# StructuralNeurobiologyLab/SyConn

Measured on AMD Instinct MI355X. Metric: segmented Mvoxels/s (whole node), 128^3 EM tiles, higher is better.
Workload: dtype bf16; 1 GPU; BASELINE configs[1]: semseg_spine 3D U-Net on 128^3 uint8 tiles, 96 tiles per GPU per step in launch sets of 8 (sd_forward_labels_batch), random-init weights, HOST TO HOST: pinned host uint8 tiles -> H2D -> kernels -> pinned host uint8 labels (stored by the last kernel, no copy), 3 HIP streams, 2 buffer sets; tiles_per_launch_set=8, parallelism=tile-sharded x1, hip_streams_per_gpu=3, collective=none

## Files before the change

syconn_amd/csrc/sd_conv_mfma.h:

```cpp
#pragma once
#include "sd_internal.h"
#include "../../include/syconn_dense.h"
#include <algorithm>
#include <cstdlib>
#include <mutex>
#include <string>
#include <type_traits>
#include <utility>

#include "sd_device.h"


template <typename T>
__device__ __forceinline__ void store_tile_rows(typename Act<T>::v4 (&o)[4], T* base, size_t P, size_t vidx, bool valid,
                                                int cbase, int half, int Cd) {
    typedef __attribute__((ext_vector_type(2))) unsigned u2;
    typedef __attribute__((ext_vector_type(4))) unsigned u4;
    u2 a0 = __builtin_bit_cast(u2, o[0]), a1 = __builtin_bit_cast(u2, o[1]);
    u2 a2 = __builtin_bit_cast(u2, o[2]), a3 = __builtin_bit_cast(u2, o[3]);
    unsigned x;
    x = a0.x; { unsigned y = a1.x; swap32(x, y); a0.x = x; a1.x = y; }
    x = a0.y; { unsigned y = a1.y; swap32(x, y); a0.y = x; a1.y = y; }
    x = a2.x; { unsigned y = a3.x; swap32(x, y); a2.x = x; a3.x = y; }
    x = a2.y; { unsigned y = a3.y; swap32(x, y); a2.y = x; a3.y = y; }
// ... 36 lines not shown
#pragma unroll
    for (int q = 0; q < 4; ++q) {
        const int n = cbase + 4 * half + 8 * q;
        f32x4 b = {0.f, 0.f, 0.f, 0.f};
        if (n < Cd) b = *reinterpret_cast<const f32x4*>(bias + n);
#pragma unroll
        for (int e = 0; e < 4; ++e) {
            float v = acc[4 * q + e] + b[e];
            if (relu) v = fmaxf(v, 0.f);
            o[q][e] = (T)v;
        }
    }
    store_tile_rows<T>(o, base, P, vidx, valid, cbase, half, Cd);
}

template <typename T>
__device__ __forceinline__ typename Act<T>::v8 gn_apply8(typename Act<T>::v8 v, const float* sc, const float* sh, int relu) {
    typedef __attribute__((ext_vector_type(4))) unsigned u4;
    const f32x4 s0 = *reinterpret_cast<const f32x4*>(sc), s1 = *reinterpret_cast<const f32x4*>(sc + 4);
    const f32x4 t0 = *reinterpret_cast<const f32x4*>(sh), t1 = *reinterpret_cast<const f32x4*>(sh + 4);
#pragma unroll
    for (int e = 0; e < 4; ++e) {
        v[e] = (T)fmaf((float)v[e], s0[e], t0[e]);
        v[4 + e] = (T)fmaf((float)v[4 + e], s1[e], t1[e]);
    }
    if (relu) {
        u4 u = __builtin_bit_cast(u4, v);
        u.x = pk_max16(u.x, 0u); u.y = pk_max16(u.y, 0u); u.z = pk_max16(u.z, 0u); u.w = pk_max16(u.w, 0u);
        v = __builtin_bit_cast(typename Act<T>::v8, u);
    }
    return v;
}

template <int KZ, int WAVES, int MT> struct ConvGeo {
    static constexpr int BZ = KZ == 3 ? (WAVES / 4) * MT : 1;
    static constexpr int BY = KZ == 3 ? 8 : WAVES * 2 * MT;
    static constexpr int BX = 16;
};


constexpr int dma_count(int w, int waves, int a_instr, int j0, int j1) {
    int n = 0;
    for (int j = j0; j < j1; ++j) n += (w + j * waves < a_instr) ? 1 : 0;
    return n;
}
constexpr int zroll_wait(int nt, int u_want, int i_want) {
    int seq = 0;
    int wseq[9] = {0, 0, 0, 0, 0, 0, 0, 0, 0};
    int xseq[3][6] = {{0}};
    seq += nt; wseq[0] = seq - 1;
    for (int m = 0; m < 4; ++m) xseq[0][m] = seq++;
    for (int u = 0; u < 9; ++u) {
        const int kx = u / 3, kz = u % 3;
        if (u + 1 < 9) { seq += nt; wseq[u + 1] = seq - 1; }
        for (int i = 0; i < 4; ++i) {
            if (u == u_want && i == i_want) {
                int need = xseq[kx][i + kz];
                if (i == 0 && wseq[u] > need) need = wseq[u];
                return seq - 1 - need;
            }
            if (kz == 0 && i == 0) xseq[kx][4] = seq++;
            else if (kz == 1 && i == 0) xseq[kx][5] = seq++;
            else if (kz == 2 && kx < 2) xseq[kx + 1][i] = seq++;
        }
    }
    return 0;
}
template <typename T, int KZ, int NT, int WAVES, int NSLOT, int MT, int MODE>
__global__ __launch_bounds__(WAVES * 64, WAVES == 12 ? 3 : 2) void k_conv_mfma(const ConvParams p) {
    constexpr bool FF = MODE == 1 || MODE == 4 || MODE == 5, GN = MODE == 2, FU8 = MODE == 5;
    constexpr bool ZROLL = KZ == 3 && NT != 3;
    if (p.clk && blockIdx.x == 0 && threadIdx.x == 0) { p.clk[0] = __builtin_readcyclecounter(); p.clk[1] = __builtin_amdgcn_s_memrealtime(); }
    constexpr bool SP = MODE == 3 || MODE == 4;
    static_assert(!SP || std::is_same<T, f16_t>::value, "split plan: fp16 planes");
    constexpr bool LEAN = MT == 4 || NT == 3;
#ifndef SD_LATE_W
#define SD_LATE_W 1
#endif
#ifdef SD_NO_SPREAD
    constexpr bool SPREAD = false;
#else
    constexpr bool SPREAD = MT == 4 && KZ == 3 && WAVES == 8 && NSLOT == 0 && (MODE == 0 || MODE == 3);
#endif
    using v8 = typename Act<T>::v8;
    using G = ConvGeo<KZ, WAVES, MT>;
    constexpr bool WRES = NSLOT > 0;
    constexpr bool RING = NSLOT < 0;
    static_assert(!RING || (KZ == 1 && MODE == 0 && MT == 2 && NSLOT == -3), "ring form: planar, plain, 2 voxel tiles per wave");
    constexpr int NA = WRES ? NSLOT : RING ? -NSLOT : 2;
    constexpr int NW = RING ? -NSLOT : 2;
    constexpr int BZ = G::BZ, BY = G::BY, BX = G::BX;
    constexpr int PZ = KZ / 2;
    constexpr int HZ = BZ + KZ - 1, HY = BY + 2, HX = BX + 2;
    constexpr int NH = HZ * HY * HX;
    constexpr int A_INSTR = (NH * 2 + 63) / 64;
    constexpr int A_BYTES = A_INSTR * 1024;
    constexpr int B_INSTR = 9 * NT;
    constexpr int B_BYTES = B_INSTR * 1024;
    constexpr int SLICE = HY * HX * 32;
    constexpr int AJ = (A_INSTR + WAVES - 1) / WAVES;
    constexpr int WJ = (B_INSTR + WAVES - 1) / WAVES;
    constexpr int WAITN = WRES ? (NA - 2) * AJ : RING ? AJ + WJ : 0;
    static_assert(WAITN < 64, "vmcnt immediate");
    extern __shared__ __attribute__((aligned(16))) char smem[];
    const int nchunks = p.nchunk0 + p.nchunk1;
    const int nstages = nchunks * KZ;
    char* const ldsA = smem;
    char* const ldsB = smem + NA * A_BYTES;
    float* const wl = reinterpret_cast<float*>(ldsB + (WRES ? nstages : NW) * B_BYTES);
    char* const fwl = reinterpret_cast<char*>(wl) + SD_CONV_PARAM_BYTES;
    char* const ldsDummy = fwl + (p.final_wfrag ? NT * 4096 : 0);
    float* const fpatch = reinterpret_cast<float*>(ldsDummy + 1024);
    float* const gnl = fpatch;

    const int tid = threadIdx.x, lane = tid & 63;
    const int wave = __builtin_amdgcn_readfirstlane(tid >> 6);
    const int nsb = p.nbx * p.nby * p.nbz;
    const int nb = blockIdx.y;
    const int gsz = gridDim.x;

    int tzs[MT], tys[MT];
#pragma unroll
    for (int i = 0; i < MT; ++i) {
        if (KZ == 3) { tzs[i] = MT * (wave >> 2) + i; tys[i] = 2 * (wave & 3); }
        else { tzs[i] = 0; tys[i] = 2 * MT * wave + 2 * i; }
    }
    const int dy = (lane & 31) >> 4, dxl = lane & 15, half = lane >> 5;
    int xoffE[MT], xoffO[MT];
#pragma unroll
    for (int i = 0; i < MT; ++i) {
        const int hv = (tzs[i] * HY + tys[i] + dy) * HX + dxl;
        xoffE[i] = hv * 32 + ((half ^ (dy & 1)) << 4);
        xoffO[i] = hv * 32 + ((half ^ (dy & 1) ^ 1) << 4);
    }

    for (int idx = tid; idx < NT * 32; idx += WAVES * 64) {
        const int n = nb * NT * 32 + idx;
        wl[idx] = n < p.Cd ? p.bias[n] : 0.f;
    }
    if constexpr (GN) {
        const int per_tile = nchunks * 32;
        for (int i = tid; i < p.batch * per_tile; i += WAVES * 64) {
            const int t = i / per_tile, r = i - t * per_tile, c = r >> 5, e = r & 31, ch = e & 15, is_shift = e >> 4;
            const bool s0 = c < p.nchunk0;
            const float* const base = s0 ? p.gn0 : p.gn1;
            const int C = s0 ? p.C0 : p.C1, cc = s0 ? c : c - p.nchunk0;
            float v = is_shift ? 0.f : 1.f;
            if (base) v = reinterpret_cast<const float*>(reinterpret_cast<const char*>(base) + (size_t)t * p.tstride)[is_shift * C + cc * SD_CHUNK + ch];
            gnl[i] = v;
        }
    }
    if (p.final_wfrag) {
        if (tid < 8) wl[NT * 32 + tid] = tid < p.final_cout ? p.final_b[tid] : 0.f;
        const T* const fwp = reinterpret_cast<const T*>(p.final_wfrag);
        for (int k = wave; k < NT * 4; k += WAVES)
            *reinterpret_cast<v8*>(fwl + (k * 64 + lane) * 16) = *reinterpret_cast<const v8*>(fwp + ((size_t)k * 64 + lane) * 8);
    }
// ... 152 lines not shown
            }
        }
    };
    int sf_c = 0, sf_round = 0, sf_slot = 0, sf_z = 0, sf_y = 0, sf_x = 0, sf_t = 0;
    bool sf_ok = false;
    auto stream_block = [&]() {
        const int lbf = block_of(sf_round);
        sf_ok = lbf >= 0;
        if (sf_ok) coords(lbf, sf_z, sf_y, sf_x, sf_t);
    };
    auto dma_stream_next = [&]() {
        if (sf_c == 0) stream_block();
        dma_halo(sf_c, sf_slot, sf_z, sf_y, sf_x, sf_t, sf_ok);
        gn_note(sf_c, sf_slot, sf_z, sf_y, sf_x, sf_t, sf_ok);
        if (++sf_c == nchunks) { sf_c = 0; ++sf_round; }
        if (++sf_slot == NA) sf_slot = 0;
    };

    auto ring_issue = [&]() {
        if (sf_c == 0) stream_block();
        const char* src = wbase + (size_t)sf_c * B_BYTES + lane * 16;
        char* dst = ldsB + sf_slot * B_BYTES;
#pragma unroll
        for (int j = 0; j < WJ; ++j) {
            const int k = wave + j * WAVES;
            const bool inst = sf_ok && k < B_INSTR;
            glds16(inst ? src + k * 1024 : reinterpret_cast<const char*>(p.zero), inst ? dst + k * 1024 : ldsDummy);
        }
        dma_halo(sf_c, sf_slot, sf_z, sf_y, sf_x, sf_t, sf_ok);
        if (++sf_c == nchunks) { sf_c = 0; ++sf_round; }
        if (++sf_slot == NA) sf_slot = 0;
    };

#ifdef SD_TIMING
    long long tstamp[8];
    long long sstamp[16];
    int tcount = 0;
#define SD_T(i) do { if (tcount == SD_TB) tstamp[i] = __builtin_readcyclecounter(); } while (0)
#else
#define SD_T(i) do {} while (0)
#endif
#ifndef SD_TS
#define SD_TS 0
#endif
#ifndef SD_TB
#define SD_TB 2
#endif
    int lb = block_of(0);
    if (lb < 0) return;
    int z0, y0, x0, tn;
    coords(lb, z0, y0, x0, tn);

    constexpr int FPX = HX + 2, FPY = HY + 2, FNP = FPX * FPY, FPT = (FNP + WAVES * 64 - 1) / (WAVES * 64);
    float fpv[FF ? FPT : 1];
    auto patch_fetch = [&](int bz0, int by0, int bx0, int btile) {
#pragma unroll
        for (int k = 0; k < FPT; ++k) {
            const int i = tid + k * WAVES * 64;
            const int px = i % FPX, py = i / FPX;
            const int y = by0 - 2 + py, x = bx0 - 2 + px;
            float v = 0.f;
            if (i < FNP && (unsigned)bz0 < (unsigned)p.D && (unsigned)y < (unsigned)p.H && (unsigned)x < (unsigned)p.W) {
                const size_t idx = ((size_t)bz0 * p.H + y) * p.W + x;
                const char* const in = reinterpret_cast<const char*>(p.first_in) + (size_t)btile * p.first_in_tstride;
                if constexpr (FU8) v = __builtin_bit_cast(float, u8_bf16_pair(reinterpret_cast<const uint8_t*>(in)[idx]));
                else if (p.first_in_f32) v = reinterpret_cast<const float*>(in)[idx];
                else v = (float)reinterpret_cast<const uint8_t*>(in)[idx] / 255.0f;
            }
            fpv[k] = v;
        }
    };
    auto patch_park = [&](int buf) {
#pragma unroll
        for (int k = 0; k < FPT; ++k) {
            const int i = tid + k * WAVES * 64;
            if (i < FNP) fpatch[buf * FNP + i] = fpv[k];
        }
    };
    constexpr int NF1 = (FF && !SP && NA == 3) ? 2 : 1;
    float* const ffw = fpatch + 2 * FNP;
    if constexpr (FF) {
        patch_fetch(z0, y0, x0, tn);
        patch_park(0);
        if constexpr (FU8) {
            if (tid == 0) reinterpret_cast<unsigned*>(ffw)[0] = SD_BF16_ONE_PAIR;
            typedef __attribute__((ext_vector_type(4))) unsigned u4;
            for (int i = tid; i < NF1 * 2 * 64; i += WAVES * 64) reinterpret_cast<u4*>(ffw + 4)[i] = reinterpret_cast<const u4*>(p.first_w3)[i];
        } else
        for (int i = tid; i < NF1 * (5 * 64 + 32); i += WAVES * 64) ffw[i] = i < NF1 * 320 ? p.first_w[i] : p.first_bias[i - NF1 * 320];
    }
    if (WRES) {
        for (int s = 0; s < nstages; ++s) dma_weights(s, s);
        if (!FF) for (int f = 0; f < NA - 1; ++f) dma_stream_next();
    } else if (RING) {
        for (int f = 0; f < NA - 1; ++f) ring_issue();
    } else {
        dma_weights(0, 0);
        dma_halo(0, 0, z0, y0, x0, tn, true);
        gn_note(0, 0, z0, y0, x0, tn, true);
    }
    if constexpr (GN) {
        static_assert(!GN || WAITN == 0, "deferred GroupNorm apply: every halo DMA is awaited at its stage end");
        asm volatile("s_waitcnt vmcnt(0) lgkmcnt(0)\n\ts_barrier" ::: "memory");
        gn_transform();
        asm volatile("s_waitcnt lgkmcnt(0)\n\ts_barrier" ::: "memory");
    } else {
        asm volatile("s_waitcnt vmcnt(%0) lgkmcnt(0)\n\ts_barrier" ::"n"(WAITN) : "memory");
    }

    StoreGuard<T> sguard;
#ifndef SD_PRIO
#define SD_PRIO 2
#endif
    if constexpr (SPREAD && SD_PRIO != 0) {
        if ((SD_PRIO == 1) == (wave >= WAVES / 2)) asm volatile("s_setprio 1");
    }
    int gc = 0, gs = 0;
    int ph0 = 0;
    if constexpr (SPREAD) {
        const int hv0 = (wave * 64 + lane) >> 1;
        ph0 = ((hv0 / (HX * HY)) << 16) | (((hv0 / HX) % HY) << 8) | (hv0 % HX);
        static_assert(!SPREAD || (HX < 256 && HY < 256), "packed piece coordinates");
    }
    constexpr int FIT = FU8 ? (NH + 32 * WAVES - 1) / (32 * WAVES) : 1;
    int fc_off[FIT], fc_yx[FIT], fc_wr = (lane & 31) * 32 + half * 8;
    if constexpr (FU8) {
#pragma unroll
        for (int it = 0; it < FIT; ++it) {
            const int hv = (wave + it * WAVES) * 32 + (lane & 31);
            const int hvc = hv < NH ? hv : NH - 1;
            const int hy = hvc / HX, hx = hvc % HX;
            fc_off[it] = (hy * (HX + 2) + hx) * 4;
            fc_yx[it] = hv < NH ? ((hy << 16) | hx) : -1;
            asm volatile("" : "+v"(fc_off[it]), "+v"(fc_yx[it]));
        }
        asm volatile("" : "+v"(fc_wr));
    }
    for (int round = 0; lb >= 0; ++round) {
        const int nlb = block_of(round + 1);
        int nz0 = 0, ny0 = 0, nx0 = 0, ntn = 0;
        if (nlb >= 0) coords(nlb, nz0, ny0, nx0, ntn);

        if constexpr (FF) {
            static_assert(!FF || (KZ == 1 && WRES && (SP ? NA == 4 : (NA == 2 || NA == 3))), "fused first conv: planar, resident weights");
            constexpr int PXW = HX + 2, NSTEP1 = 5;
            const float* const fp = fpatch + (round & 1) * FNP;
            if constexpr (FU8) {
                const unsigned* const up = reinterpret_cast<const unsigned*>(fp);
                const unsigned* const cpair = reinterpret_cast<const unsigned*>(ffw);
                const bf16x8* const w3l = reinterpret_cast<const bf16x8*>(ffw + 4);
                bf16x8 w30 = w3l[lane], w31 = w3l[64 + lane];
                int toff5[5];
#pragma unroll
                for (int a = 0; a < 5; ++a) {
                    const int tap = half * 5 + a;
// ... 110 lines not shown
                }
                }
            }
            }
            asm volatile("s_waitcnt lgkmcnt(0)\n\ts_barrier" ::: "memory");
            if (nlb >= 0) patch_fetch(nz0, ny0, nx0, ntn);
        }
        f32x16 acc[MT][NT];
#pragma unroll
        for (int i = 0; i < MT; ++i)
#pragma unroll
            for (int j = 0; j < NT; ++j)
#pragma unroll
                for (int r = 0; r < 16; ++r) acc[i][j][r] = wl[j * 32 + 4 * half + 8 * (r >> 2) + (r & 3)];
#ifdef SD_TIMING
        ++tcount;
#endif
        SD_T(0);
#ifdef SD_RT
        const long long rt0 = __builtin_amdgcn_s_memrealtime();
#endif
        int s = 0;
        for (int c = 0; c < nchunks; ++c, ++gc) {
            const char* const abuf = ldsA + ((SP && FF) ? (c < 4 ? (c & 1) : c - 2) : (gc % NA)) * A_BYTES;
            bool pf_real = false;
            const char* pf_sbase = nullptr;
            const char* pf_zero = reinterpret_cast<const char*>(p.zero);
            char* pf_dst = nullptr;
            int pf_Hs = 0, pf_Ws = 0, pf_z = 0, pf_y = 0, pf_x = 0, pf_D = p.D, pf_H = p.H, pf_W = p.W;
            auto pf_setup = [&]() {
                int pc = c + 1, pt = tn;
                pf_real = true; pf_z = z0; pf_y = y0; pf_x = x0;
                if (pc == nchunks) { pc = 0; pt = ntn; pf_z = nz0; pf_y = ny0; pf_x = nx0; pf_real = nlb >= 0; }
                size_t Ps;
                int pn;
                if (pc < p.nchunk0) { pf_sbase = (const char*)p.src0; Ps = p.P0; pf_Hs = p.H0; pf_Ws = p.W0; pn = p.nchunk0; }
                else { pf_sbase = (const char*)p.src1; Ps = p.P1; pf_Hs = p.H1; pf_Ws = p.W1; pc -= p.nchunk0; pn = p.nchunk1; }
                if constexpr (SP) { if (pc >= pn / 3) pc -= pn / 3; }
                pf_sbase += (size_t)pc * Ps * (SD_CHUNK * sizeof(T)) + (size_t)pt * p.tstride;
                pf_z -= PZ; pf_y -= 1; pf_x -= 1;
                pf_dst = ldsA + ((gc + 1) & 1) * A_BYTES + wave * 1024;
                auto rfl = [](int v) { return __builtin_amdgcn_readfirstlane(v); };
                {
                    const uint64_t a = reinterpret_cast<uint64_t>(pf_sbase);
                    pf_sbase = reinterpret_cast<const char*>(((uint64_t)(unsigned)rfl((int)(a >> 32)) << 32) | (unsigned)rfl((int)a));
                }
                pf_Hs = rfl(pf_Hs); pf_Ws = rfl(pf_Ws); pf_z = rfl(pf_z); pf_y = rfl(pf_y); pf_x = rfl(pf_x);
                asm volatile("" : "+s"(pf_sbase), "+s"(pf_zero), "+s"(pf_Hs), "+s"(pf_Ws), "+s"(pf_z), "+s"(pf_y), "+s"(pf_x),
                             "+s"(pf_D), "+s"(pf_H), "+s"(pf_W));
            };
            (void)pf_setup;
            if constexpr (SPREAD) pf_setup();
            constexpr int SV = WAVES * 32, SDZ = SV / (HY * HX), SDY = (SV % (HY * HX)) / HX, SDX = SV % HX;
            static_assert(SDY + 1 <= HY && SDX < HX, "piece stride");
            int ph_x = ph0 & 255, ph_y = (ph0 >> 8) & 255, ph_z = ph0 >> 16;
            auto dma_piece = [&](int j) {
                const int k = wave + j * WAVES;
                if (pf_real && j < AJ && k < A_INSTR) {
                    const int idx = k * 64 + lane;
                    const int z = pf_z + ph_z, y = pf_y + ph_y, x = pf_x + ph_x;
                    const bool ok = idx < NH * 2 && (unsigned)z < (unsigned)pf_D && (unsigned)y < (unsigned)pf_H &&
                                    (unsigned)x < (unsigned)pf_W;
                    const unsigned vox = ((unsigned)z * (unsigned)pf_Hs + (unsigned)y) * (unsigned)pf_Ws + (unsigned)x;
                    const unsigned hf = ((unsigned)(lane ^ ph_y) & 1u) << 4;
                    const uint64_t off = ((uint64_t)(vox >> 27) << 32) | ((vox << 5) | hf);
                    const char* src = pf_zero;
                    if (ok) src = pf_sbase + off;
                    glds16(src, pf_dst + j * (WAVES * 1024));
                }
                ph_x += SDX;
                if (ph_x >= HX) { ph_x -= HX; ++ph_y; }
                ph_y += SDY;
                if (ph_y >= HY) { ph_y -= HY; ++ph_z; }
                ph_z += SDZ;
            };
            constexpr int EB = (AJ + 2) / 3, LB = (AJ + 1) / 2;
            constexpr int E0 = dma_count(WAVES - 1, WAVES, A_INSTR, 0, EB), E1 = dma_count(WAVES - 1, WAVES, A_INSTR, EB, 2 * EB);
            constexpr int L0 = dma_count(WAVES / 2 - 1, WAVES, A_INSTR, 0, LB), L1 = dma_count(WAVES / 2 - 1, WAVES, A_INSTR, LB, 2 * LB);
            static_assert(!SPREAD || (3 * EB >= AJ && 2 * LB >= AJ), "halo piece schedule");
            auto halo_pieces = [&](int j0, int n) {
                for (int j = j0; j < j0 + n; ++j) dma_piece(j);
            };
#pragma unroll 1
            for (int kz = 0; kz < KZ; ++kz, ++s, ++gs) {
                if (s == SD_TS) SD_T(7);
                if constexpr (RING) {
                    if (wave >= WAVES / 2) ring_issue();
                } else if (!WRES) {
                    if (!(SPREAD && SD_LATE_W) || wave >= WAVES / 2 || s + 1 == nstages) {
                        if (s + 1 < nstages) dma_weights(s + 1, (gs + 1) & 1);
                        else if (nlb >= 0) dma_weights(0, (gs + 1) & 1);
                    }
                    if constexpr (SPREAD) {
                        if (wave >= WAVES / 2) halo_pieces(kz * EB, EB);
                    }
                    if (!SPREAD && kz == 0) {
                        if (c + 1 < nchunks) {
                            dma_halo(c + 1, (gc + 1) & 1, z0, y0, x0, tn, true);
                            gn_note(c + 1, (gc + 1) & 1, z0, y0, x0, tn, true);
                        } else if (nlb >= 0) {
                            dma_halo(0, (gc + 1) & 1, nz0, ny0, nx0, ntn, true);
                            gn_note(0, (gc + 1) & 1, nz0, ny0, nx0, ntn, true);
                        }
                    }
                } else if (kz == 0 && !FF) {
                    dma_stream_next();
                }
                constexpr bool GN_ASYNC = GN && KZ == 3 && !WRES;
                if constexpr (GN_ASYNC) {
                    if (kz == 1 && wave < WAVES / 2) { gn_transform(); asm volatile("s_waitcnt lgkmcnt(0)" ::: "memory"); }
                }
                if (s == SD_TS) SD_T(1);
                const char* const bcur = ldsB + (WRES ? s : RING ? gs % NW : (gs & 1)) * B_BYTES + lane * 16;
                const char* const acur = ZROLL ? abuf + kz * (HX * 32) : abuf + kz * SLICE;
                const bool odd_row = ZROLL && (kz & 1);
                if constexpr (MT == 4 && ZROLL) {
                    v8 xq[4], wq[2][NT];
                    const uint32_t bA = lds_addr(bcur);
                    const uint32_t xb = lds_addr(acur) + (odd_row ? xoffO[0] : xoffE[0]);
// ... 79 lines not shown
                    static_for<NT>([&](auto jc) {
                        constexpr int j = decltype(jc)::value;
                        ds_read16<(t9 * NT + j) * 1024>(wf[buf][j], bA);
                    });
                };
                load_tap(std::integral_constant<int, 0>{});
                static_for<9>([&](auto tc) {
                    constexpr int t9 = decltype(tc)::value, buf = t9 & 1;
                    if constexpr (t9 + 1 < 9) {
                        load_tap(std::integral_constant<int, t9 + 1>{});
                        asm volatile("s_waitcnt lgkmcnt(%0)" ::"n"(MT + NT));
                    } else {
                        asm volatile("s_waitcnt lgkmcnt(0)");
                    }
#pragma unroll
                    for (int i = 0; i < MT; ++i) tie(xf[buf][i]);
#pragma unroll
                    for (int j = 0; j < NT; ++j) tie(wf[buf][j]);
#pragma unroll
                    for (int i = 0; i < MT; ++i)
#pragma unroll
                        for (int j = 0; j < NT; ++j)
                            acc[i][j] = Act<T>::mfma(wf[buf][j], xf[buf][i], acc[i][j]);
                });
                }
                if (s == SD_TS) SD_T(2);
                if constexpr (GN_ASYNC) {
                    if (kz == 1 && wave >= WAVES / 2) gn_transform();
                    asm volatile("s_waitcnt vmcnt(0) lgkmcnt(0)\n\ts_barrier" ::: "memory");
                } else if constexpr (GN) {
                    asm volatile("s_waitcnt vmcnt(0) lgkmcnt(0)" ::: "memory");
                    gn_transform();
                    asm volatile("s_waitcnt lgkmcnt(0)\n\ts_barrier" ::: "memory");
                } else if constexpr (RING) {
                    if (wave < WAVES / 2) ring_issue();
                    asm volatile("s_waitcnt vmcnt(%0) lgkmcnt(0)\n\ts_barrier" ::"n"(WAITN) : "memory");
                } else if constexpr (SPREAD) {
                    const bool late = wave < WAVES / 2;
                    if (SD_LATE_W && late && s + 1 < nstages) dma_weights(s + 1, (gs + 1) & 1);
                    if (late && kz < 2) halo_pieces(kz * LB, LB);
                    const int fly = !pf_real || kz == 2 ? 0 : late ? (kz == 0 ? L0 : L1) : (kz == 0 ? E0 : E1);
                    static_assert(!SPREAD || (E0 <= 4 && E1 <= 4 && L0 <= 4 && L1 <= 4), "counted waits below");
                    if (fly == 4) asm volatile("s_waitcnt vmcnt(4) lgkmcnt(0)\n\ts_barrier" ::: "memory");
                    else if (fly == 3) asm volatile("s_waitcnt vmcnt(3) lgkmcnt(0)\n\ts_barrier" ::: "memory");
                    else if (fly == 2) asm volatile("s_waitcnt vmcnt(2) lgkmcnt(0)\n\ts_barrier" ::: "memory");
                    else if (fly == 1) asm volatile("s_waitcnt vmcnt(1) lgkmcnt(0)\n\ts_barrier" ::: "memory");
                    else if (s + 1 == nstages && !p.gn_sums) {
                        asm volatile("s_waitcnt vmcnt(0) lgkmcnt(0)" ::: "memory");
                    }
                    else asm volatile("s_waitcnt vmcnt(0) lgkmcnt(0)\n\ts_barrier" ::: "memory");
                } else {
                    asm volatile("s_waitcnt vmcnt(%0) lgkmcnt(0)\n\ts_barrier" ::"n"(WAITN) : "memory");
                }
                if constexpr (FF) {
                    if (s == 0 && nlb >= 0) patch_park((round + 1) & 1);
                }
                if (s == SD_TS) SD_T(3);
#ifdef SD_STAGES
                if (tcount == SD_TB && s < 14) sstamp[s] = __builtin_readcyclecounter();
#endif
            }
        }

    SD_T(4);
    if constexpr (SP) {
        T* const dsts = reinterpret_cast<T*>(reinterpret_cast<char*>(p.dst) + (size_t)tn * p.tstride);
// ... 55 lines not shown
                            d = Act<T>::mfma(__builtin_bit_cast(v8, h1), s2, d);
#pragma unroll
                            for (int r = 0; r < 16; ++r) { sj += d[r]; ssj = fmaf(d[r], d[r], ssj); }
                        }
                    }
                }
                if (p.pool_dst) {
                    unsigned ph[8], pl[8];
#pragma unroll
                    for (int k = 0; k < 8; ++k) {
                        float a = -INFINITY, b = -INFINITY;
#pragma unroll
                        for (int e2 = 0; e2 < NP; ++e2) {
                            float ae = acc[ip + e2][j][2 * k] * osc, be = acc[ip + e2][j][2 * k + 1] * osc;
                            if (p.relu) { ae = fmaxf(ae, 0.f); be = fmaxf(be, 0.f); }
                            a = fmaxf(a, vals[e2] ? ae : -INFINITY);
                            b = fmaxf(b, vals[e2] ? be : -INFINITY);
                        }
                        a = max_xor16(max_xor1(a));
                        b = max_xor16(max_xor1(b));
                        split_pk(a, b, ph[k], pl[k]);
                    }
                    const int pz = (KZ == 3) ? (z0 + tzs[ip]) >> 1 : z0 + tzs[ip], py = (y0 + tys[ip]) >> 1, px = (x0 + dxl) >> 1;
                    const size_t po = (size_t)(pz * p.pH + py) * p.pW + px;
                    const bool writer = (dy == 0) && ((dxl & 1) == 0) && vals[0];
                    store_tile_rows_pk<T>(ph, pdsts, p.Pp, po, writer, (nb * NT + j) * 32, half, p.Cd);
                    store_tile_rows_pk<T>(pl, pdstl, p.Pp, po, writer, (nb * NT + j) * 32, half, p.Cd);
                }
            }
            if (gns) {
                float* const q = part + ((size_t)(wave * 2 + half) * (NT * 32) + j * 32 + (lane & 31)) * 2;
                q[0] = sj; q[1] = ssj;
            }
            if constexpr (SPREAD) {
                if (j == 0 && wave >= WAVES / 2 && !p.gn_sums) asm volatile("s_barrier" ::: "memory");
            }
        }
        if (gns) {
            __syncthreads();
            if (tid < NT * 64) {
                const int stat = tid / (NT * 32), cw = tid % (NT * 32);
                double t = 0.0;
                for (int w = 0; w < WAVES * 2; ++w) t += (double)part[((size_t)w * (NT * 32) + cw) * 2 + stat];
                const int ch = nb * NT * 32 + cw;
                if (ch < p.Cd)
                    atomicAdd(reinterpret_cast<double*>(reinterpret_cast<char*>(p.gn_sums) + (size_t)tn * p.tstride) +
                                  (size_t)stat * p.gn_C + ch, t);
            }
            __syncthreads();
        }
        if constexpr (MT == 2 && KZ == 1) {
        if (p.final_wfrag) {
            const FinalOut fo{p.final_out, p.out_tstride, p.final_cout, p.final_kind, p.final_nvox, p.ovf};
            typedef __attribute__((ext_vector_type(4))) unsigned u4;
#pragma unroll
            for (int tp = 0; tp < MT; tp += 2) {
                f32x16 lgt[2];
                bool vv[2];
                size_t vo2[2];
#pragma unroll
                for (int i = 0; i < 2; ++i) {
                    const int vz = z0 + tzs[tp + i], vy = y0 + tys[tp + i] + dy, vx = x0 + dxl;
                    vv[i] = vz < p.D && vy < p.H && vx < p.W;
                    vo2[i] = (size_t)(vz * p.Hd + vy) * p.Wd + vx;
#pragma unroll
                    for (int r = 0; r < 16; ++r) lgt[i][r] = 0.f;
#pragma unroll
// ... 85 lines not shown
                    }
                    if (p.store_main)
                        store_tile_rows_pk_at<T>(pk2[e2], qj + (size_t)(ip + e2) * (vzs * SD_CHUNK), cstr, val2[e2], cj0, cj1);
                }
                if (p.pool_dst) {
                    T* const pdst = reinterpret_cast<T*>(reinterpret_cast<char*>(p.pool_dst) + (size_t)tn * p.tstride);
                    const bool writer = (dy == 0) && ((dxl & 1) == 0);
                    if constexpr (KZ == 3) {
                        unsigned m[8];
#pragma unroll
                        for (int k = 0; k < 8; ++k) m[k] = pk_max16(val2[0] ? pk2[0][k] : 0u, val2[1] ? pk2[1][k] : 0u);
                        pool_xy_pk8(m);
                        const int pz = (vz0 + ip) >> 1, py = (y0 + tys[0]) >> 1, px = (x0 + dxl) >> 1;
                        store_tile_rows_pk<T>(m, pdst, p.Pp, (size_t)(pz * p.pH + py) * p.pW + px, writer && val2[0],
                                              (nb * NT + j) * 32, half, p.Cd);
                    } else {
#pragma unroll
                        for (int e2 = 0; e2 < 2; ++e2) {
                            unsigned m[8];
#pragma unroll
                            for (int k = 0; k < 8; ++k) m[k] = val2[e2] ? pk2[e2][k] : 0u;
                            pool_xy_pk8(m);
                            const int py = (y0 + tys[ip + e2]) >> 1, px = (x0 + dxl) >> 1;
                            store_tile_rows_pk<T>(m, pdst, p.Pp, (size_t)(vz0 * p.pH + py) * p.pW + px, writer && val2[e2],
                                                  (nb * NT + j) * 32, half, p.Cd);
                        }
                    }
                }
            }
            if (p.gn_sums) {
                float* const q = part + ((size_t)(wave * 2 + half) * (NT * 32) + j * 32 + (lane & 31)) * 2;
                q[0] = sj; q[1] = ssj;
            }
            if constexpr (SPREAD) {
                if (j == 0 && wave >= WAVES / 2 && !p.gn_sums) asm volatile("s_barrier" ::: "memory");
            }
        }
        if (p.gn_sums) {
            __syncthreads();
            if (tid < NT * 64) {
                const int stat = tid / (NT * 32), cw = tid % (NT * 32);
                double t = 0.0;
                for (int w = 0; w < WAVES * 2; ++w) t += (double)part[((size_t)w * (NT * 32) + cw) * 2 + stat];
                const int ch = nb * NT * 32 + cw;
                if (ch < p.Cd)
                    atomicAdd(reinterpret_cast<double*>(reinterpret_cast<char*>(p.gn_sums) + (size_t)tn * p.tstride) +
                                  (size_t)stat * p.gn_C + ch, t);
            }
            __syncthreads();
        }
    } else {
    bool valid[MT];
    size_t voxoff[MT];
#pragma unroll
    for (int i = 0; i < MT; ++i) {
        const int vz = z0 + tzs[i], vy = y0 + tys[i] + dy, vx = x0 + dxl;
        valid[i] = vz < p.D && vy < p.H && vx < p.W;
        voxoff[i] = (size_t)(vz * p.Hd + vy) * p.Wd + vx;
    }
    T* const dst = reinterpret_cast<T*>(reinterpret_cast<char*>(p.dst) + (size_t)tn * p.tstride);
    unsigned pk[MT][NT][8];
#pragma unroll
    for (int i = 0; i < MT; ++i)
#pragma unroll
        for (int j = 0; j < NT; ++j)
#pragma unroll
            for (int k = 0; k < 8; ++k)
// ... 179 lines not shown
            } else {
                guard = logit_probe<T>(l, p.final_cout);
            }
            const bool vmine = half ? valid[tp + 1] : valid[tp];
            if (vmine) range_guard<T>(guard, p.ovf);
            const size_t v = half ? voxoff[tp + 1] : voxoff[tp];
            if (vmine) {
                if (p.final_kind == SD_OUT_LABELS_U8) {
                    uint8_t lab = 0;
                    for (int k = 0; k < p.lab.n; ++k) {
                        const int id = p.lab.ids[k];
                        float pv = 0.f;
#pragma unroll
                        for (int co = 0; co < 8; ++co) pv = (co == id) ? l[co] : pv;
                        if ((int)(uint8_t)(pv * 255.f) >= p.lab.cuts[k]) lab = (uint8_t)id;
                    }
                    (reinterpret_cast<uint8_t*>(p.final_out) + (size_t)tn * p.out_tstride)[v] = lab;
                } else if (p.final_kind == SD_OUT_PROBS_U8) {
                    uint8_t* out = reinterpret_cast<uint8_t*>(p.final_out) + (size_t)tn * p.out_tstride;
#pragma unroll
                    for (int co = 0; co < 8; ++co)
                        if (co < p.final_cout) out[(size_t)co * nvox + v] = (uint8_t)(l[co] * 255.f);
                } else {
                    float* out = reinterpret_cast<float*>(reinterpret_cast<char*>(p.final_out) + (size_t)tn * p.out_tstride);
#pragma unroll
                    for (int co = 0; co < 8; ++co)
                        if (co < p.final_cout) out[(size_t)co * nvox + v] = l[co];
                }
            }
        }
    }

    }
        if constexpr (SPREAD) {
            if (wave < WAVES / 2 && !p.gn_sums) asm volatile("s_barrier" ::: "memory");
        }
        SD_T(6);
#ifdef SD_TIMING
        if (tcount == SD_TB && lane == 0 && p.dbg) {
            long long* o = p.dbg + ((size_t)blockIdx.x * WAVES + wave) * 8;
            for (int i = 0; i < 8; ++i) o[i] = tstamp[i];
#ifdef SD_STAGES
            sstamp[14] = tstamp[0]; sstamp[15] = tstamp[6];
            long long* o2 = p.dbg + (1 << 20) + ((size_t)blockIdx.x * WAVES + wave) * 16;
            for (int i = 0; i < 16; ++i) o2[i] = sstamp[i];
#endif
#ifdef SD_RT
            o[4] = rt0; o[5] = __builtin_amdgcn_s_memrealtime();
            o[6] = ((long long)__builtin_amdgcn_s_getreg((31 << 11) | 20) << 32) | (unsigned)__builtin_amdgcn_s_getreg((31 << 11) | 4);
#endif
        }
#endif
        lb = nlb; z0 = nz0; y0 = ny0; x0 = nx0; tn = ntn;
    }
    if (p.clk && blockIdx.x == 0 && threadIdx.x == 0) { p.clk[2] = __builtin_readcyclecounter(); p.clk[3] = __builtin_amdgcn_s_memrealtime(); }
    sguard.flush(p.ovf);
}

static inline int grid_for(long total, int per_block = 256, int cap = 256 * 16) {
    long g = (total + per_block - 1) / per_block;
    if (g > cap) g = cap;
    if (g < 1) g = 1;
    return (int)g;
}
#define SD_LAUNCH_CHECK() (hipGetLastError() == hipSuccess ? SD_OK : SD_ERR_HIP)

constexpr int SD_LDS_BYTES = 160 * 1024;
constexpr int SD_NUM_CU = 256;
constexpr int SD_MAX_DEVICES = 64;
struct LaunchCache { size_t attr_set = 0, occ_lds = 0; int occ = 1; };

template <int KZ, int NT, int WAVES, int MT, int NSLOT>
static size_t conv_lds_bytes(int nstages, bool fuse_final = false) {
    using G = ConvGeo<KZ, WAVES, MT>;
    constexpr int NH = (G::BZ + KZ - 1) * (G::BY + 2) * (G::BX + 2);
    constexpr int A_BYTES = (NH * 2 + 63) / 64 * 1024;
    return (size_t)(NSLOT > 0 ? NSLOT : NSLOT < 0 ? -NSLOT : 2) * A_BYTES + (size_t)(NSLOT > 0 ? nstages : NSLOT < 0 ? -NSLOT : 2) * 9 * NT * 1024 +
           SD_CONV_PARAM_BYTES + (fuse_final ? NT * 4096 : 0) + 1024;
}

template <typename T, int KZ, int NT, int WAVES, int NSLOT, int MT = 2, int MODE = 0>
static int launch_conv_k(ConvParams p, int NB, hipStream_t s) {
    using G = ConvGeo<KZ, WAVES, MT>;
    constexpr bool FF = MODE == 1 || MODE == 4 || MODE == 5;
    const size_t lds = conv_lds_bytes<KZ, NT, WAVES, MT, NSLOT>((p.nchunk0 + p.nchunk1) * KZ, p.final_wfrag != nullptr) +
                       (FF ? (size_t)2 * (G::BY + 4) * (G::BX + 4) * 4 + (MODE == 5 ? (size_t)16 + (NSLOT == 3 ? 2 : 1) * 2048
                                                                                      : (size_t)(MODE == 1 && NSLOT == 3 ? 2 : 1) * (5 * 64 + 32) * 4) : 0) +
                       (MODE == 2 ? (size_t)p.batch * conv_gn_lds_per_tile(p.nchunk0 + p.nchunk1) : 0);
    if (lds > (size_t)SD_LDS_BYTES) return SD_ERR_INVALID;
    p.nbx = (p.W + G::BX - 1) / G::BX; p.nby = (p.H + G::BY - 1) / G::BY; p.nbz = (p.D + G::BZ - 1) / G::BZ;
    if (const char* ns = getenv("SD_TIMING_NO_STORE")) {
        if (KZ == 3 || atoi(ns) >= 2) { p.store_main = 0; p.pool_dst = nullptr; }
    }
    static const int order = getenv("SD_BLOCK_ORDER") ? atoi(getenv("SD_BLOCK_ORDER")) : 1;
    p.block_order = order;
    auto kern = k_conv_mfma<T, KZ, NT, WAVES, NSLOT, MT, MODE>;
    static std::mutex mu;
    static LaunchCache cache[SD_MAX_DEVICES];
    int occ = 1;
    {
        int dev = 0;
        if (hipGetDevice(&dev) != hipSuccess || dev < 0 || dev >= SD_MAX_DEVICES) return SD_ERR_HIP;
        std::lock_guard<std::mutex> lock(mu);
        LaunchCache& c = cache[dev];
        if (lds > c.attr_set) {
            if (hipFuncSetAttribute(reinterpret_cast<const void*>(kern), hipFuncAttributeMaxDynamicSharedMemorySize,
                                    (int)lds) != hipSuccess) return SD_ERR_HIP;
            c.attr_set = lds;
        }
        if (lds != c.occ_lds) {
            int n = 0;
            if (hipOccupancyMaxActiveBlocksPerMultiprocessor(&n, reinterpret_cast<const void*>(kern), WAVES * 64, lds) !=
                hipSuccess) n = 1;
            c.occ = std::max(1, n);
            c.occ_lds = lds;
        }
        occ = c.occ;
    }
    const int nsb = p.nbx * p.nby * p.nbz * p.batch;
    const int wg_per_cu = std::min(occ, (int)(SD_LDS_BYTES / lds));
    const int cap = std::max(8, SD_NUM_CU * wg_per_cu / NB / 8 * 8);
    static const bool no_persist = getenv("SD_NO_PERSIST") != nullptr;
    dim3 grid(!no_persist ? std::min(nsb, cap) : nsb, NB), block(WAVES * 64);
    {
        static const std::string name = std::string("k_conv_mfma<") + (std::is_same<T, bf16_t>::value ? "bf16" : "f16") + "," +
            std::to_string(KZ) + "x3x3,NT=" + std::to_string(NT) + ",WAVES=" + std::to_string(WAVES) + ",NSLOT=" + std::to_string(NSLOT) +
            ",MT=" + std::to_string(MT) + ",MODE=" + std::to_string(MODE) + ">";
        SD_NOTE_KERNEL(name.c_str());
    }
    hipLaunchKernelGGL(kern, grid, block, lds, s, p);
    return SD_LAUNCH_CHECK();
}
```

syconn_amd/csrc/sd_kernels.hip:

```cpp
#include "sd_internal.h"
#include "../../include/syconn_dense.h"
#include <algorithm>
#include <cstdlib>
#include <mutex>
#include <string>
#include <type_traits>
#include <utility>

#include "sd_device.h"

#include "sd_conv_mfma.h"


template <typename T, int KZ, typename IN, bool SPLIT = false>
__global__ __launch_bounds__(256) void k_conv_first(const FirstParams p) {
    constexpr int BZ = sd_bz(KZ), BY = sd_by(KZ), BX = SD_BX;
    constexpr int PZ = KZ / 2;
    constexpr int HZ = BZ + KZ - 1, HY = BY + 2, HX = BX + 2;
    constexpr int NH = HZ * HY * HX;
    constexpr int NTAP = KZ * 9;
    constexpr int NSTEP = (NTAP + 1) / 2;
    __shared__ float patch[NH];

    const int tid = threadIdx.x, lane = tid & 63, wave = tid >> 6;
// ... 1036 lines not shown
    const long vox = (long)p.D * p.H * p.W * (p.batch_total > 0 ? p.batch_total : p.batch);
    const int nstages = (p.nchunk0 + p.nchunk1) * KZ;
    const char* const big_env = getenv("SD_BIG_MIN");
    const long big_min = big_env ? atol(big_env) : 256;
    const bool big = (vox / 512) * NB >= big_min && !(KZ == 1 && NT == 3 && !getenv("SD_PLANAR_NT3_BIG"));
    if constexpr (KZ == 1 && NT <= 2) {
        if (p.first_in) {
            if (!conv_can_fuse_first(KZ, NT, NB, vox, nstages, p.final_wfrag != nullptr)) return SD_ERR_INVALID;
            if (p.first_w3 && !p.first_in_f32) {
                if constexpr (NT == 2) {
                    if (nstages == 3) return launch_conv_k<T, KZ, NT, 8, 3, 2, 5>(p, NB, s);
                }
                return launch_conv_k<T, KZ, NT, 8, 2, 2, 5>(p, NB, s);
            }
            if constexpr (NT == 2) {
                if (nstages == 3) return launch_conv_k<T, KZ, NT, 8, 3, 2, 1>(p, NB, s);
            }
            return launch_conv_k<T, KZ, NT, 8, 2, 2, 1>(p, NB, s);
        }
    } else if (p.first_in) {
        return SD_ERR_INVALID;
    }
    if (p.gn0 || p.gn1) {
        const size_t gl = (size_t)p.batch * conv_gn_lds_per_tile(p.nchunk0 + p.nchunk1);
        if (big) {
            const char* const gcap_env = getenv("SD_WRES_GN_CAP_KB");
            const size_t gn_cap = (size_t)(gcap_env ? atoi(gcap_env) : ((long)p.D * p.H * p.W >= (1l << 20) ? 158 : 80)) * 1024;
            if (conv_lds_bytes<KZ, NT, 8, 2, 2>(nstages, p.final_wfrag != nullptr) + gl <= gn_cap) return launch_conv_k<T, KZ, NT, 8, 2, 2, 2>(p, NB, s);
            return launch_conv_k<T, KZ, NT, 8, 0, 2, 2>(p, NB, s);
        }
        if (conv_lds_bytes<KZ, NT, 4, 2, 2>(nstages, p.final_wfrag != nullptr) + gl <= 80 * 1024) return launch_conv_k<T, KZ, NT, 4, 2, 2, 2>(p, NB, s);
        return launch_conv_k<T, KZ, NT, 4, 0, 2, 2>(p, NB, s);
    }
    if (big) {
        const char* const cap_env = getenv("SD_WRES_CAP_KB");
        const size_t wres_cap = (size_t)(cap_env ? atoi(cap_env) : ((long)p.D * p.H * p.W >= (1l << 20) ? 150 : 96)) * 1024;
        if (conv_lds_bytes<KZ, NT, 8, 2, 2>(nstages, p.final_wfrag != nullptr) <= wres_cap) return launch_conv_k<T, KZ, NT, 8, 2>(p, NB, s);
        if constexpr (KZ == 3 && NT == 2) {
            const bool mt2 = getenv("SD_MT2") != nullptr;
            const bool z_ok = getenv("SD_MT4_D_RULE") ? (p.D % 8 == 0 || p.D >= 96) : ((p.D + 7) / 8 * 8) * 100 <= ((p.D + 3) / 4 * 4) * 105;
            if (!mt2 && !p.final_wfrag && (vox / 1024) * NB >= 256 && z_ok)
                return launch_conv_k<T, KZ, NT, 8, 0, 4>(p, NB, s);
        }
        if constexpr (KZ == 1 && NT == 2) {
            const bool no_p4 = getenv("SD_NO_PLANAR4") != nullptr;
            if (!no_p4 && !p.final_wfrag && (p.H % 32 == 0 || p.H >= 128 || !getenv("SD_PLANAR4_H_RULE")) && (vox / 512) * NB >= 1024)
                return launch_conv_k<T, KZ, NT, 4, 0, 4>(p, NB, s);
        }
        if constexpr (KZ == 1 && NT == 3) {
            const bool no_ring = getenv("SD_NO_RING") != nullptr;
            if (!no_ring && nstages >= 3 && conv_lds_bytes<KZ, NT, 8, 2, -3>(nstages, p.final_wfrag != nullptr) <= (size_t)SD_LDS_BYTES)
                return launch_conv_k<T, KZ, NT, 8, -3>(p, NB, s);
        }
        return launch_conv_k<T, KZ, NT, 8, 0>(p, NB, s);
    }
    if (conv_lds_bytes<KZ, NT, 4, 2, 2>(nstages, p.final_wfrag != nullptr) <= 80 * 1024) return launch_conv_k<T, KZ, NT, 4, 2>(p, NB, s);
    return launch_conv_k<T, KZ, NT, 4, 0>(p, NB, s);
}
template <typename T>
static int launch_conv2_t(const ConvParams& p, int KZ, int NT, int NB, hipStream_t s) {
    if (KZ == 3 && NT == 3) return launch_conv_knt<T, 3, 3>(p, NB, s);
    if (KZ == 1 && NT == 3) return launch_conv_knt<T, 1, 3>(p, NB, s);
    if (KZ == 3 && NT == 2) return launch_conv_knt<T, 3, 2>(p, NB, s);
    if (KZ == 3 && NT == 1) return launch_conv_knt<T, 3, 1>(p, NB, s);
    if (KZ == 1 && NT == 2) return launch_conv_knt<T, 1, 2>(p, NB, s);
    if (KZ == 1 && NT == 1) return launch_conv_knt<T, 1, 1>(p, NB, s);
    return SD_ERR_INVALID;
}
int launch_conv(const ConvParams& p, int act_dtype, int KZ, int NT, int NB, hipStream_t s) {
    if (act_dtype == SD_F16X2) return launch_conv_split(p, KZ, NT, NB, s);
    return act_dtype == SD_BF16 ? launch_conv2_t<bf16_t>(p, KZ, NT, NB, s) : launch_conv2_t<f16_t>(p, KZ, NT, NB, s);
}

template <typename T, typename IN>
static int launch_first_t(const FirstParams& p, int KZ, hipStream_t s) {
    SD_NOTE_KERNEL(sizeof(IN) == 1 ? (p.wpack3 && KZ == 1 ? "k_conv_first<uint8 input, bf16 MFMA on the exact values>" : "k_conv_first<uint8 input, f32 MFMA chain>")
                                   : "k_conv_first<float32 input, f32 MFMA chain>");
// ... 351 lines not shown
```

Baseline: 3077 Mvox/s.

## Add 8-wave 4-tile planar ring conv variant with split weight/halo DMA waves

Adds a new planar (KZ=1, NT=2) conv form that uses 8 waves with 4 voxel tiles each over a 2x32x16 block. It keeps a 3-slot halo ring and double-buffers weights, which are streamed only by the upper half of the waves, while halo pieces are spread across both halves with asymmetric priorities and barriers. It becomes the default for large planar layers when the shape fits (D even, H a multiple of 32, enough work, LDS fits), replacing the 4-wave planar4 path. The aim is more reuse per staged weight slice and better overlap of DMA with MFMA, at the cost of larger per-workgroup LDS and possibly lower occupancy. It also adds an environment cap on the persistent grid size.

```diff
diff --git a/syconn_amd/csrc/sd_conv_mfma.h b/syconn_amd/csrc/sd_conv_mfma.h
--- a/syconn_amd/csrc/sd_conv_mfma.h
+++ b/syconn_amd/csrc/sd_conv_mfma.h
@@ -92,9 +92,10 @@
     return v;
 }
 
-template <int KZ, int WAVES, int MT> struct ConvGeo {
-    static constexpr int BZ = KZ == 3 ? (WAVES / 4) * MT : 1;
-    static constexpr int BY = KZ == 3 ? 8 : WAVES * 2 * MT;
+template <int KZ, int WAVES, int MT, int NSLOT = 0> struct ConvGeo {
+    static constexpr bool P8 = KZ == 1 && WAVES == 8 && MT == 4 && NSLOT < 0;
+    static constexpr int BZ = KZ == 3 ? (WAVES / 4) * MT : P8 ? 2 : 1;
+    static constexpr int BY = KZ == 3 ? 8 : P8 ? 32 : WAVES * 2 * MT;
     static constexpr int BX = 16;
 };
 
@@ -143,12 +144,14 @@
     constexpr bool SPREAD = MT == 4 && KZ == 3 && WAVES == 8 && NSLOT == 0 && (MODE == 0 || MODE == 3);
 #endif
     using v8 = typename Act<T>::v8;
-    using G = ConvGeo<KZ, WAVES, MT>;
+    using G = ConvGeo<KZ, WAVES, MT, NSLOT>;
     constexpr bool WRES = NSLOT > 0;
     constexpr bool RING = NSLOT < 0;
-    static_assert(!RING || (KZ == 1 && MODE == 0 && MT == 2 && NSLOT == -3), "ring form: planar, plain, 2 voxel tiles per wave");
+    constexpr bool P8 = RING && MT == 4;
+    static_assert(!RING || (KZ == 1 && MODE == 0 && NSLOT == -3 && (MT == 2 || (MT == 4 && WAVES == 8 && NT == 2))),
+                  "ring form: planar, plain, 2 voxel tiles per wave or the 8-wave 4-tile form");
     constexpr int NA = WRES ? NSLOT : RING ? -NSLOT : 2;
-    constexpr int NW = RING ? -NSLOT : 2;
+    constexpr int NW = (RING && !P8) ? -NSLOT : 2;
     constexpr int BZ = G::BZ, BY = G::BY, BX = G::BX;
     constexpr int PZ = KZ / 2;
     constexpr int HZ = BZ + KZ - 1, HY = BY + 2, HX = BX + 2;
@@ -159,8 +162,9 @@
     constexpr int B_BYTES = B_INSTR * 1024;
     constexpr int SLICE = HY * HX * 32;
     constexpr int AJ = (A_INSTR + WAVES - 1) / WAVES;
-    constexpr int WJ = (B_INSTR + WAVES - 1) / WAVES;
-    constexpr int WAITN = WRES ? (NA - 2) * AJ : RING ? AJ + WJ : 0;
+    constexpr int WIW = P8 ? WAVES / 2 : WAVES;
+    constexpr int WJ = (B_INSTR + WIW - 1) / WIW;
+    constexpr int WAITN = WRES ? (NA - 2) * AJ : P8 ? AJ : RING ? AJ + WJ : 0;
     static_assert(WAITN < 64, "vmcnt immediate");
     extern __shared__ __attribute__((aligned(16))) char smem[];
     const int nchunks = p.nchunk0 + p.nchunk1;
@@ -183,6 +187,7 @@
 #pragma unroll
     for (int i = 0; i < MT; ++i) {
         if (KZ == 3) { tzs[i] = MT * (wave >> 2) + i; tys[i] = 2 * (wave & 3); }
+        else if (P8) { tzs[i] = wave >> 2; tys[i] = 2 * MT * (wave & 3) + 2 * i; }
         else { tzs[i] = 0; tys[i] = 2 * MT * wave + 2 * i; }
     }
     const int dy = (lane & 31) >> 4, dxl = lane & 15, half = lane >> 5;
@@ -401,6 +406,23 @@
         if (++sf_slot == NA) sf_slot = 0;
     };
 
+    auto p8_weights = [&](int sidx, int slot) {
+        const char* src = wbase + (size_t)(sidx < 0 ? 0 : sidx) * B_BYTES + lane * 16;
+        char* dst = ldsB + slot * B_BYTES;
+#pragma unroll
+        for (int j = 0; j < WJ; ++j) {
+            const int k = (wave - WAVES / 2) + j * (WAVES / 2);
+            const bool inst = sidx >= 0 && k < B_INSTR;
+            glds16(inst ? src + k * 1024 : reinterpret_cast<const char*>(p.zero), inst ? dst + k * 1024 : ldsDummy);
+        }
+    };
+    auto ring_halo_issue = [&]() {
+        if (sf_c == 0) stream_block();
+        dma_halo(sf_c, sf_slot, sf_z, sf_y, sf_x, sf_t, sf_ok);
+        if (++sf_c == nchunks) { sf_c = 0; ++sf_round; }
+        if (++sf_slot == NA) sf_slot = 0;
+    };
+
 #ifdef SD_TIMING
     long long tstamp[8];
     long long sstamp[16];
@@ -461,6 +483,9 @@
     if (WRES) {
         for (int s = 0; s < nstages; ++s) dma_weights(s, s);
         if (!FF) for (int f = 0; f < NA - 1; ++f) dma_stream_next();
+    } else if (P8) {
+        if (wave >= WAVES / 2) p8_weights(0, 0);
+        for (int f = 0; f < NA - 1; ++f) ring_halo_issue();
     } else if (RING) {
         for (int f = 0; f < NA - 1; ++f) ring_issue();
     } else {
@@ -481,15 +506,16 @@
 #ifndef SD_PRIO
 #define SD_PRIO 2
 #endif
-    if constexpr (SPREAD && SD_PRIO != 0) {
+    constexpr bool ASYM = SPREAD || P8;
+    if constexpr (ASYM && SD_PRIO != 0) {
         if ((SD_PRIO == 1) == (wave >= WAVES / 2)) asm volatile("s_setprio 1");
     }
     int gc = 0, gs = 0;
     int ph0 = 0;
-    if constexpr (SPREAD) {
+    if constexpr (ASYM) {
         const int hv0 = (wave * 64 + lane) >> 1;
         ph0 = ((hv0 / (HX * HY)) << 16) | (((hv0 / HX) % HY) << 8) | (hv0 % HX);
-        static_assert(!SPREAD || (HX < 256 && HY < 256), "packed piece coordinates");
+        static_assert(!ASYM || (HX < 256 && HY < 256), "packed piece coordinates");
     }
     constexpr int FIT = FU8 ? (NH + 32 * WAVES - 1) / (32 * WAVES) : 1;
     int fc_off[FIT], fc_yx[FIT], fc_wr = (lane & 31) * 32 + half * 8;
@@ -666,6 +692,13 @@
                 int pc = c + 1, pt = tn;
                 pf_real = true; pf_z = z0; pf_y = y0; pf_x = x0;
                 if (pc == nchunks) { pc = 0; pt = ntn; pf_z = nz0; pf_y = ny0; pf_x = nx0; pf_real = nlb >= 0; }
+                int pslot = (gc + 1) & 1;
+                if constexpr (P8) {
+                    if (sf_c == 0) stream_block();
+                    pc = sf_c; pt = sf_t; pf_z = sf_z; pf_y = sf_y; pf_x = sf_x; pf_real = sf_ok; pslot = sf_slot;
+                    if (++sf_c == nchunks) { sf_c = 0; ++sf_round; }
+                    if (++sf_slot == NA) sf_slot = 0;
+                }
                 size_t Ps;
                 int pn;
                 if (pc < p.nchunk0) { pf_sbase = (const char*)p.src0; Ps = p.P0; pf_Hs = p.H0; pf_Ws = p.W0; pn = p.nchunk0; }
@@ -673,7 +706,7 @@
                 if constexpr (SP) { if (pc >= pn / 3) pc -= pn / 3; }
                 pf_sbase += (size_t)pc * Ps * (SD_CHUNK * sizeof(T)) + (size_t)pt * p.tstride;
                 pf_z -= PZ; pf_y -= 1; pf_x -= 1;
-                pf_dst = ldsA + ((gc + 1) & 1) * A_BYTES + wave * 1024;
+                pf_dst = ldsA + pslot * A_BYTES + wave * 1024;
                 auto rfl = [](int v) { return __builtin_amdgcn_readfirstlane(v); };
                 {
                     const uint64_t a = reinterpret_cast<uint64_t>(pf_sbase);
@@ -684,7 +717,7 @@
                              "+s"(pf_D), "+s"(pf_H), "+s"(pf_W));
             };
             (void)pf_setup;
-            if constexpr (SPREAD) pf_setup();
+            if constexpr (ASYM) pf_setup();
             constexpr int SV = WAVES * 32, SDZ = SV / (HY * HX), SDY = (SV % (HY * HX)) / HX, SDX = SV % HX;
             static_assert(SDY + 1 <= HY && SDX < HX, "piece stride");
             int ph_x = ph0 & 255, ph_y = (ph0 >> 8) & 255, ph_z = ph0 >> 16;
@@ -701,6 +734,8 @@
                     const char* src = pf_zero;
                     if (ok) src = pf_sbase + off;
                     glds16(src, pf_dst + j * (WAVES * 1024));
+                } else if constexpr (P8) {
+                    if (j < AJ) glds16(pf_zero, ldsDummy);
                 }
                 ph_x += SDX;
                 if (ph_x >= HX) { ph_x -= HX; ++ph_y; }
@@ -718,7 +753,12 @@
 #pragma unroll 1
             for (int kz = 0; kz < KZ; ++kz, ++s, ++gs) {
                 if (s == SD_TS) SD_T(7);
-                if constexpr (RING) {
+                if constexpr (P8) {
+                    if (wave >= WAVES / 2) {
+                        p8_weights(s + 1 < nstages ? s + 1 : (nlb >= 0 ? 0 : -1), (gs + 1) & 1);
+                        halo_pieces(0, AJ);
+                    }
+                } else if constexpr (RING) {
                     if (wave >= WAVES / 2) ring_issue();
                 } else if (!WRES) {
                     if (!(SPREAD && SD_LATE_W) || wave >= WAVES / 2 || s + 1 == nstages) {
@@ -864,6 +904,10 @@
                     asm volatile("s_waitcnt vmcnt(0) lgkmcnt(0)" ::: "memory");
                     gn_transform();
                     asm volatile("s_waitcnt lgkmcnt(0)\n\ts_barrier" ::: "memory");
+                } else if constexpr (P8) {
+                    if (wave < WAVES / 2) halo_pieces(0, AJ);
+                    if (s + 1 == nstages && !p.gn_sums) asm volatile("s_waitcnt vmcnt(%0) lgkmcnt(0)" ::"n"(WAITN) : "memory");
+                    else asm volatile("s_waitcnt vmcnt(%0) lgkmcnt(0)\n\ts_barrier" ::"n"(WAITN) : "memory");
                 } else if constexpr (RING) {
                     if (wave < WAVES / 2) ring_issue();
                     asm volatile("s_waitcnt vmcnt(%0) lgkmcnt(0)\n\ts_barrier" ::"n"(WAITN) : "memory");
@@ -985,7 +1029,7 @@
                 float* const q = part + ((size_t)(wave * 2 + half) * (NT * 32) + j * 32 + (lane & 31)) * 2;
                 q[0] = sj; q[1] = ssj;
             }
-            if constexpr (SPREAD) {
+            if constexpr (ASYM) {
                 if (j == 0 && wave >= WAVES / 2 && !p.gn_sums) asm volatile("s_barrier" ::: "memory");
             }
         }
@@ -1137,7 +1181,7 @@
                 float* const q = part + ((size_t)(wave * 2 + half) * (NT * 32) + j * 32 + (lane & 31)) * 2;
                 q[0] = sj; q[1] = ssj;
             }
-            if constexpr (SPREAD) {
+            if constexpr (ASYM) {
                 if (j == 0 && wave >= WAVES / 2 && !p.gn_sums) asm volatile("s_barrier" ::: "memory");
             }
         }
@@ -1383,7 +1427,7 @@
     }
 
     }
-        if constexpr (SPREAD) {
+        if constexpr (ASYM) {
             if (wave < WAVES / 2 && !p.gn_sums) asm volatile("s_barrier" ::: "memory");
         }
         SD_T(6);
@@ -1423,16 +1467,16 @@
 
 template <int KZ, int NT, int WAVES, int MT, int NSLOT>
 static size_t conv_lds_bytes(int nstages, bool fuse_final = false) {
-    using G = ConvGeo<KZ, WAVES, MT>;
+    using G = ConvGeo<KZ, WAVES, MT, NSLOT>;
     constexpr int NH = (G::BZ + KZ - 1) * (G::BY + 2) * (G::BX + 2);
     constexpr int A_BYTES = (NH * 2 + 63) / 64 * 1024;
-    return (size_t)(NSLOT > 0 ? NSLOT : NSLOT < 0 ? -NSLOT : 2) * A_BYTES + (size_t)(NSLOT > 0 ? nstages : NSLOT < 0 ? -NSLOT : 2) * 9 * NT * 1024 +
+    return (size_t)(NSLOT > 0 ? NSLOT : NSLOT < 0 ? -NSLOT : 2) * A_BYTES + (size_t)(NSLOT > 0 ? nstages : (NSLOT < 0 && !G::P8) ? -NSLOT : 2) * 9 * NT * 1024 +
            SD_CONV_PARAM_BYTES + (fuse_final ? NT * 4096 : 0) + 1024;
 }
 
 template <typename T, int KZ, int NT, int WAVES, int NSLOT, int MT = 2, int MODE = 0>
 static int launch_conv_k(ConvParams p, int NB, hipStream_t s) {
-    using G = ConvGeo<KZ, WAVES, MT>;
+    using G = ConvGeo<KZ, WAVES, MT, NSLOT>;
     constexpr bool FF = MODE == 1 || MODE == 4 || MODE == 5;
     const size_t lds = conv_lds_bytes<KZ, NT, WAVES, MT, NSLOT>((p.nchunk0 + p.nchunk1) * KZ, p.final_wfrag != nullptr) +
                        (FF ? (size_t)2 * (G::BY + 4) * (G::BX + 4) * 4 + (MODE == 5 ? (size_t)16 + (NSLOT == 3 ? 2 : 1) * 2048
@@ -1470,7 +1514,8 @@
     }
     const int nsb = p.nbx * p.nby * p.nbz * p.batch;
     const int wg_per_cu = std::min(occ, (int)(SD_LDS_BYTES / lds));
-    const int cap = std::max(8, SD_NUM_CU * wg_per_cu / NB / 8 * 8);
+    int cap = std::max(8, SD_NUM_CU * wg_per_cu / NB / 8 * 8);
+    if (const char* const wc = getenv("SD_CONV_WGS_CAP")) cap = std::max(8, std::min(cap, atoi(wc) / 8 * 8));
     static const bool no_persist = getenv("SD_NO_PERSIST") != nullptr;
     dim3 grid(!no_persist ? std::min(nsb, cap) : nsb, NB), block(WAVES * 64);
     {
diff --git a/syconn_amd/csrc/sd_kernels.hip b/syconn_amd/csrc/sd_kernels.hip
--- a/syconn_amd/csrc/sd_kernels.hip
+++ b/syconn_amd/csrc/sd_kernels.hip
@@ -1092,6 +1092,16 @@
         if (conv_lds_bytes<KZ, NT, 4, 2, 2>(nstages, p.final_wfrag != nullptr) + gl <= 80 * 1024) return launch_conv_k<T, KZ, NT, 4, 2, 2, 2>(p, NB, s);
         return launch_conv_k<T, KZ, NT, 4, 0, 2, 2>(p, NB, s);
     }
+    bool p8_default = false;
+    (void)p8_default;
+    if constexpr (KZ == 1 && NT == 2) {
+        const char* const p8_env = getenv("SD_PLANAR8");
+        const int p8 = p8_env ? (atoi(p8_env) == 0 ? 0 : 2) : 1;
+        const bool p8_geo = !p.final_wfrag && nstages >= 4 &&
+                            conv_lds_bytes<KZ, NT, 8, 4, -3>(nstages, false) <= (size_t)SD_LDS_BYTES;
+        if (p8 == 2 && p8_geo) return launch_conv_k<T, KZ, NT, 8, -3, 4>(p, NB, s);
+        p8_default = p8 == 1 && p8_geo && (vox / 1024) * NB >= 256 && p.D % 2 == 0 && p.H % 32 == 0;
+    }
     if (big) {
         const char* const cap_env = getenv("SD_WRES_CAP_KB");
         const size_t wres_cap = (size_t)(cap_env ? atoi(cap_env) : ((long)p.D * p.H * p.W >= (1l << 20) ? 150 : 96)) * 1024;
@@ -1103,6 +1113,9 @@
                 return launch_conv_k<T, KZ, NT, 8, 0, 4>(p, NB, s);
         }
         if constexpr (KZ == 1 && NT == 2) {
+            if constexpr (NT == 2) {
+                if (p8_default) return launch_conv_k<T, KZ, NT, 8, -3, 4>(p, NB, s);
+            }
             const bool no_p4 = getenv("SD_NO_PLANAR4") != nullptr;
             if (!no_p4 && !p.final_wfrag && (p.H % 32 == 0 || p.H >= 128 || !getenv("SD_PLANAR4_H_RULE")) && (vox / 512) * NB >= 1024)
                 return launch_conv_k<T, KZ, NT, 4, 0, 4>(p, NB, s);
```

After: 3086 Mvox/s, median of 6. About the same (+0.3%).
